# marcin-ochman/modular-slam

Hardware: AMD Instinct MI355X
Metric: ORB keypoints extracted+matched /sec, 640×480 RGB-D, 1/2/4/8 GPU; HBM GB/s vs roofline (higher is better)
Workload: dtype u8

## Files before the change

### modular-slam_amd/csrc/api.hip

```cpp
#include "context.hpp"

#include <cfloat>
#include <climits>
#include <cmath>
#include <cstdio>
#include <cstring>
#include <cstdlib>
#include <algorithm>

using namespace mslam;

static thread_local std::string g_create_error;

#define HIPCHK(c, call)                                                                                                \
    do                                                                                                                 \
    {                                                                                                                  \
        hipError_t e_ = (call);                                                                                        \
        if(e_ != hipSuccess)                                                                                           \
        {                                                                                                              \
            (c)->err = std::string(#call) + ": " + hipGetErrorString(e_);                                              \
            return MSLAM_HIP_E_RUNTIME;                                                                                \
        }                                                                                                              \
    } while(0)

// ... 290 lines not shown
void mslam_hip_default_params(mslam_hip_params* p)
{
    std::memset(p, 0, sizeof(*p));
    p->width = 640;
    p->height = 480;
    p->max_batch = 1;
    p->n_levels = 8;
    p->scale_factor = 1.2f;
    p->ini_fast_thr = 20;
    p->min_fast_thr = 7;
    p->min_node_area = 1000;
    p->max_keypoints = 8192;
    p->max_candidates = 16384;
    p->device = 0;
    p->stream = nullptr;
    p->detector = MSLAM_HIP_DETECTOR_DISTRIBUTED;
    p->n_features = 1000;
    p->edge_threshold = 31;
}

int mslam_hip_abi_version(void) { return MSLAM_HIP_ABI_VERSION; }

const char* mslam_hip_last_error(const mslam_hip_ctx* ctx) { return ctx ? ctx->err.c_str() : g_create_error.c_str(); }

void mslam_hip_destroy(mslam_hip_ctx* c)
{
    if(!c)
        return;
    if(c->stream)
        (void)hipStreamSynchronize(c->stream);
    void* bufs[] = {c->d_cells,   c->d_rs_ofs, c->d_rs_coef, c->d_rs_qt, c->d_ratio_thr, c->d_orient_w, c->d_stage,  c->d_pyr,
                    c->d_blur,    c->d_cv_ofs, c->d_cv_coef, c->d_cell_cnt, c->d_cell_kp, c->quad.cand, c->quad.cand_cnt, c->quad.sel,
                    c->quad.sel_cnt, c->quad.kp_node, c->quad.nodes_a, c->quad.nodes_b, c->quad.ncnt_a, c->quad.ncnt_b,
                    c->quad.child_cnt, c->quad.ninfo, c->quad.best, c->d_flags, c->d_hm_from, c->d_hm_out, c->d_hm_partial,
                    c->d_xyz, c->d_valid, c->d_pnp_obj, c->d_pnp_img, c->d_pnp_n, c->d_pnp_counts, c->d_pnp_hyp, c->d_pnp_out,
                    c->d_pnp_mask, c->d_blur_waves, c->d_pnp1_obj, c->d_pnp1_img, c->d_pnp1_hyp, c->d_pnp1_out,
                    c->d_pnp1_counts, c->d_pnp1_mask, c->d_mse1};
    for(void* b : bufs)
        if(b)
            (void)hipFree(b);
    if(c->h_out)
        (void)hipHostFree(c->h_out);
    if(c->h_hm)
        (void)hipHostFree(c->h_hm);
    if(c->h_stage)
        (void)hipHostFree(c->h_stage);
    if(c->match_graph)
        (void)hipGraphExecDestroy(c->match_graph);
    for(auto& e : c->detect_graph)
        if(e)
            (void)hipGraphExecDestroy(e);
    if(c->stream_m)
        (void)hipStreamSynchronize(c->stream_m);
    for(auto& o : c->out)
    {
        void* ob[] = {o.xy, o.desc, o.octave, o.angle, o.response, o.count, o.idx0, o.idx1, o.dist0, o.dist1, o.mfrom, o.mto, o.mcount};
        for(void* b : ob)
            if(b)
                (void)hipFree(b);
        if(o.ev_detect)
            (void)hipEventDestroy(o.ev_detect);
        if(o.ev_match)
            (void)hipEventDestroy(o.ev_match);
    }
    if(c->stream_m)
        (void)hipStreamDestroy(c->stream_m);
    for(auto& t : c->timers)
// ... 272 lines not shown
                              (double)B * g.slab < 4294901760.0  && (size_t)B * (p.width / 4) < (1u << 22) && p.height >= 8;
            int n_fused = fits ? 1 : 0;
            while(n_fused >= 1 && n_fused < p.n_levels && c->rs_q[n_fused] != SIZE_MAX && g.lv[n_fused].h >= 8 &&
                  (size_t)B * ((g.lv[n_fused].w + 3) / 4) < (1u << 22))
                ++n_fused;
            c->fused_levels = std::max(0, std::min(want, n_fused));
            const char* t = getenv("MSLAM_HIP_TILED_BLUR");
            c->geom.blur_tiled = c->fused_levels == p.n_levels && !(t && atoi(t) == 0) ? 1 : 0;
        }
        std::vector<BlurWave> bw;
        build_blur_waves(g, c->fused_levels, bw);
        c->blur_wpf = (int)bw.size();
        if(!bw.empty())
        {
            HIPCHK(c, dmalloc(c->d_blur_waves, bw.size()));
            HIPCHK(c, hipMemcpy(c->d_blur_waves, bw.data(), bw.size() * sizeof(BlurWave), hipMemcpyHostToDevice));
        }
    }
    HIPCHK(c, dmalloc(c->d_cell_cnt, B * g.n_cells));
    HIPCHK(c, dmalloc(c->d_cell_kp, B * g.n_cells * (size_t)kCellCap));
    QuadArgs& q = c->quad;
    HIPCHK(c, dmalloc(q.cand, B * L * cap));
    HIPCHK(c, dmalloc(q.cand_cnt, B * L));
    HIPCHK(c, dmalloc(q.sel, B * L * cap));
    HIPCHK(c, dmalloc(q.sel_cnt, B * L));
    HIPCHK(c, dmalloc(q.kp_node, B * L * cap));
    HIPCHK(c, dmalloc(q.nodes_a, B * L * cap));
    HIPCHK(c, dmalloc(q.nodes_b, B * L * cap));
    HIPCHK(c, dmalloc(q.ncnt_a, B * L * cap));
    HIPCHK(c, dmalloc(q.ncnt_b, B * L * cap));
    HIPCHK(c, dmalloc(q.child_cnt, B * L * cap * 4));
    HIPCHK(c, dmalloc(q.ninfo, B * L * cap));
    HIPCHK(c, dmalloc(q.best, B * L * cap));
    q.cell_cnt = c->d_cell_cnt;
    q.cell_kp = c->d_cell_kp;
    q.flags = c->d_flags;
    q.cand_cap = p.max_candidates;
    q.min_size = p.min_node_area;
    }

    for(auto& o : c->out)
    {
        HIPCHK(c, dmalloc(o.xy, (B + 1) * K * 2));
        HIPCHK(c, dmalloc(o.desc, (B + 1) * K * 32));
        HIPCHK(c, dmalloc(o.octave, (B + 1) * K));
        HIPCHK(c, dmalloc(o.angle, (B + 1) * K));
        HIPCHK(c, dmalloc(o.response, (B + 1) * K));
        HIPCHK(c, dmalloc(o.count, B + 1));
        HIPCHK(c, hipMemset(o.count, 0, (B + 1) * 4));
        HIPCHK(c, dmalloc(o.idx0, B * K));
        HIPCHK(c, dmalloc(o.idx1, B * K));
        HIPCHK(c, dmalloc(o.dist0, B * K));
        HIPCHK(c, dmalloc(o.dist1, B * K));
        HIPCHK(c, dmalloc(o.mfrom, B * K));
        HIPCHK(c, dmalloc(o.mto, B * K));
        HIPCHK(c, dmalloc(o.mcount, B));
        HIPCHK(c, hipMemset(o.mcount, 0, B * 4));
        HIPCHK(c, hipEventCreateWithFlags(&o.ev_detect, hipEventDisableTiming));
        HIPCHK(c, hipEventCreateWithFlags(&o.ev_match, hipEventDisableTiming));
    }
    HIPCHK(c, hipStreamCreateWithFlags(&c->stream_m, hipStreamNonBlocking));
    {
        const char* e = getenv("MSLAM_HIP_OVERLAP_MATCH");
        c->overlap_match = !(e && atoi(e) == 0);
        auto on = [](const char* name) { const char* v = getenv(name); return !v || atoi(v) != 0; };
        c->knob_mirror_results = on("MSLAM_HIP_MIRROR_RESULTS");
        c->knob_zero_copy = on("MSLAM_HIP_ZERO_COPY_FRAME");
        c->knob_match_graph = on("MSLAM_HIP_MATCH_GRAPH");
        const char* zm = getenv("MSLAM_HIP_ZERO_COPY_MAX_BYTES");
        c->zero_copy_max_bytes = zm ? (size_t)atoll(zm) : (size_t)1200000;
        const char* m = getenv("MSLAM_HIP_MATCHER");
// ... 329 lines not shown
        else if(blur_needed)
        {
            StageScope t(c, "blur", cs);
            launch_blur(c->d_pyr, c->d_blur, g, c->d_blur_waves, c->blur_wpf, f0, nf, cs);
        }
        }
        if(cv_mode && c->fused_levels < g.n_levels)
        {
            StageScope t(c, "blur", cs);
            launch_blur(c->d_pyr, c->d_blur, g, c->d_blur_waves, c->blur_wpf, f0, nf, cs);
        }
        {
            StageScope t(c, "describe", cs);
            DescArgs a{};
            a.pyr = c->d_pyr;
            a.blur = c->d_blur;
            a.sel = c->quad.sel;
            a.sel_cnt = c->quad.sel_cnt;
            a.orient_w = c->d_orient_w;
            a.cand_cap = c->p.max_candidates;
            a.max_kp = c->p.max_keypoints;
            a.xy = c->d_xy + K * 2;
            a.desc = c->d_desc + K * 32;
            a.octave = c->d_octave + K;
            a.angle = c->d_angle + K;
            a.response = c->d_response + K;
            a.count = c->d_count + 1;
            a.flags = c->d_flags;
            if(cv_mode)
            {
                a.sel_resp = reinterpret_cast<const float*>(c->quad.best);
                a.cv_mode = 1;
            }
            if(c->mirror_results && n_frames == 1)
                a.h_mirror = c->d_h_out;
            launch_describe(g, a, f0, nf, cs);
        }
        if(n_chunks > 1)
        {
            HIPCHK(c, hipEventRecord(c->ev_join[k], cs));
            HIPCHK(c, hipStreamWaitEvent(s, c->ev_join[k], 0));
        }
    }
    HIPCHK(c, hipGetLastError());
    return MSLAM_HIP_OK;
}

static int detect_prologue(mslam_hip_ctx* c)
{
    const size_t K = (size_t)c->p.max_keypoints;
    hipStream_t s = c->stream;
    if(!c->inplace_timing)
        c->timers_used = 0;
    if(c->n_last > 0)
    {
        const int prev = c->cur, nxt = prev ^ 1;
        if(c->out[nxt].match_pending)
        {
            HIPCHK(c, hipStreamWaitEvent(s, c->out[nxt].ev_match, 0));
            c->out[nxt].match_pending = false;
        }
        const size_t last = (size_t)c->n_last;
        hipLaunchKernelGGL(k_carry_prev, dim3(16), dim3(256), 0, s, reinterpret_cast<uint4*>(c->out[nxt].desc),
                           reinterpret_cast<const uint4*>(c->out[prev].desc + last * K * 32), c->out[nxt].count,
                           c->out[prev].count + last, (int)K);
        HIPCHK(c, hipGetLastError());
// ... 646 lines not shown
```

### modular-slam_amd/csrc/common.hpp

```cpp
#pragma once
#include <hip/hip_runtime.h>
#include <cstdint>
#include <cstddef>

namespace mslam
{

constexpr int kMaxLevels = 16;
constexpr int kBorder = 19;
constexpr int kCell = 64;
constexpr int kOverlap = 6;
constexpr int kCellCap = 1024;

struct LevelGeom
{
    int w, h;
    int pitch;
    int offset;
    float scale;
    int bw, bh;
    int cell_base;
    int n_cells;
    int bsx;
    int nxg, nyg;
// ... 66 lines not shown
    const uint4* qt;
    const int32_t* yofs;
    const uint32_t* ycoef;
    int frame0, n_frames;
    int quads;
    float inv_quads;
    int R;
    int need_mask;
    int exact;
};
void launch_resize_col(const ResizeColArgs& a, hipStream_t s);
void launch_fast(const uint8_t* d_pyr, const Geometry& g, const CellDesc* d_cells, uint32_t* d_cell_cnt,
                 uint32_t* d_cell_kp, int ini_thr, int min_thr, int frame0, int n_frames, hipStream_t s);
void launch_denorm_selfcheck(uint32_t* d_out, hipStream_t s);
struct QuadArgs
{
    const uint32_t* cell_cnt;
    const uint32_t* cell_kp;
    uint32_t* cand;
    uint32_t* cand_cnt;
    uint32_t* sel;
    uint32_t* sel_cnt;
    uint32_t* kp_node;
    uint2* nodes_a;
    uint2* nodes_b;
    uint32_t* ncnt_a;
    uint32_t* ncnt_b;
    uint32_t* child_cnt;
    uint32_t* ninfo;
    uint32_t* best;
    uint32_t* flags;
    int cand_cap;
    unsigned min_size;
};
void launch_quadtree(const Geometry& g, const QuadArgs& a, int frame0, int n_frames, hipStream_t s);
struct BlurK
{
    uint32_t ta[3], tb[4], tc[4];
    uint32_t t01, t23, t45, t6;
};
BlurK make_blur_k();
struct GrayBlurArgs
{
    const uint8_t* bgr;
    uint8_t* pyr;
    uint8_t* blur;
    int W, H, pitch;
    unsigned slab;
    int n_frames, frame0;
    int quads;
    float inv_quads;
    int k6;
    int waves_per_xcd;
    int blur_tiled;
    BlurK bk;
};
void launch_gray_blur(const GrayBlurArgs& a, hipStream_t s);
struct ResizeBlurArgs
{
    uint8_t* pyr;
    uint8_t* blur;
    unsigned slab;
    int src_off, sh, spitch, dst_off, dw, dh, dpitch;
    const uint4* qt;
    const int32_t* yofs;
    const uint32_t* ycoef;
// ... 17 lines not shown
    int n_lv;
    int G;
    int n_groups, groups_per_xcd;
    int frame0, n_frames;
};
bool launch_level_chain(const GrayBlurArgs& g, const ResizeBlurArgs* lv, int n_lv, int frames_per_group, int waves, int k6_max, hipStream_t s);
struct BlurWave
{
    int level;
    int item0;
    int generic;
    float inv_bsx;
};
void launch_blur(const uint8_t* d_pyr, uint8_t* d_blur, const Geometry& g, const BlurWave* d_waves, int wpf, int frame0, int n_frames,
                 hipStream_t s);
struct DescArgs
{
    const uint8_t* pyr;
    const uint8_t* blur;
    const uint32_t* sel;
    const uint32_t* sel_cnt;
    const uint32_t* orient_w;
    int cand_cap;
    int max_kp;
    float* xy;
    uint8_t* desc;
    int32_t* octave;
    float* angle;
    float* response;
    int32_t* count;
    uint32_t* flags;
    int n_frames = 0;
    const float* sel_resp = nullptr;
    uint8_t* h_mirror = nullptr;
    int cv_mode = 0;
};
void launch_describe(const Geometry& g, const DescArgs& a, int frame0, int n_frames, hipStream_t s);

struct ExactResizeArgs
{
    uint8_t* pyr;
    unsigned slab;
    int src_off, sw, sh, spitch, dst_off, dw, dh, dpitch;
    const int32_t* xofs;
    const uint32_t* xcoef;
    const int32_t* yofs;
    const uint32_t* ycoef;
    int xmin, xmax, ymin, ymax;
    int window12;
    int frame0;
};
void launch_resize_exact(const ExactResizeArgs& a, int n_frames, hipStream_t s);
struct CvSelectArgs
{
    uint32_t* cand;
    uint32_t* cand_cnt;
    uint32_t* tmp_kp;
    float* tmp_resp;
    uint32_t* sel;
    float* sel_resp;
    uint32_t* sel_cnt;
    uint32_t* flags;
    int cand_cap;
    int edge;
    int quota[kMaxLevels];
    int std_order;
// ... 46 lines not shown
```

### modular-slam_amd/csrc/k_describe.hip

```cpp
#include "common.hpp"
#include <cstdlib>
#include <type_traits>
#include "../../include/mslam_orb_pattern.h"
#include "../../include/mslam_sincos.h"

namespace mslam
{

__constant__ __attribute__((aligned(16))) float c_pattern_f[1024] = MSLAM_ORB_PATTERN_INIT;

__device__ __forceinline__ float fast_atan2_deg(float y, float x)
{
    constexpr float scale = (float)(180 / 3.1415926535897932384626433832795);
    constexpr float p1 = 0.9997878412794807f * scale, p3 = -0.3258083974640975f * scale;
    constexpr float p5 = 0.1555786518463281f * scale, p7 = -0.04432655554792128f * scale;
    const float ax = fabsf(x), ay = fabsf(y);
    const float eps = (float)2.2204460492503131e-16;
    float a, c, c2;
    if(ax >= ay)
        c = __fdiv_rn(ay, __fadd_rn(ax, eps));
    else
        c = __fdiv_rn(ax, __fadd_rn(ay, eps));
    c2 = __fmul_rn(c, c);
    a = __fadd_rn(__fmul_rn(p7, c2), p5);
    a = __fadd_rn(__fmul_rn(a, c2), p3);
    a = __fadd_rn(__fmul_rn(a, c2), p1);
    a = __fmul_rn(a, c);
    if(!(ax >= ay))
        a = __fsub_rn(90.f, a);
    if(x < 0)
        a = __fsub_rn(180.f, a);
    if(y < 0)
        a = __fsub_rn(360.f, a);
    return a;
}

__device__ __forceinline__ float poly_cos(float v)
{
    const float c1 = 0.99940307f, c2 = -0.49558072f, c3 = 0.03679168f;
    const float v2 = __fmul_rn(v, v);
    return __fadd_rn(c1, __fmul_rn(v2, __fadd_rn(c2, __fmul_rn(c3, v2))));
}
__device__ __forceinline__ float util_cos(float v)
{
    constexpr float PI = 3.14159265358979f;
    constexpr float PI_2 = PI / 2.0f, TWO_PI = 2.0f * PI, INV_TWO_PI = 1.0f / TWO_PI, THREE_PI_2 = 3.0f * PI_2;
    v = __fsub_rn(v, __fmul_rn((float)(int)floorf(__fmul_rn(v, INV_TWO_PI)), TWO_PI));
    v = (0.0f < v) ? v : -v;
    if(v < PI_2)
        return poly_cos(v);
    else if(v < PI)
        return -poly_cos(__fsub_rn(PI, v));
    else if(v < THREE_PI_2)
        return -poly_cos(__fsub_rn(v, PI));
    else
        return poly_cos(__fsub_rn(TWO_PI, v));
}
__device__ __forceinline__ float util_sin(float v)
{
    constexpr float PI_2 = 3.14159265358979f / 2.0f;
    return util_cos(__fsub_rn(PI_2, v));
}

constexpr int kPatchR = 18;
constexpr int kPatchRows = 2 * kPatchR + 1;
constexpr int kPatchRowsT = kPatchRows + 1;
constexpr int kPatchDw = 12;
#ifndef MSLAM_DISC_DW
#define MSLAM_DISC_DW 16
#endif
constexpr int kPatchDwT = 16;
constexpr int kPatchBufsT = 4;
constexpr int kPatchBufs = 5;
constexpr int kBlocksPerFrame = 32;

__device__ __forceinline__ uint32_t write_lane(uint32_t dst, uint32_t val, int sel)
{
    uint32_t keep_m0;
    asm volatile("s_mov_b32 %1, m0\n\ts_mov_b32 m0, %3\n\ts_nop 4\n\tv_writelane_b32 %0, %2, m0\n\ts_mov_b32 m0, %1"
                 : "+v"(dst), "=&s"(keep_m0)
                 : "s"(val), "s"(sel));
    return dst;
}

__device__ __forceinline__ int wave_sum_dpp(int v)
{
    v += __builtin_amdgcn_update_dpp(0, v, 0x111, 0xF, 0xF, true);
    v += __builtin_amdgcn_update_dpp(0, v, 0x112, 0xF, 0xF, true);
    v += __builtin_amdgcn_update_dpp(0, v, 0x114, 0xF, 0xE, true);
    v += __builtin_amdgcn_update_dpp(0, v, 0x118, 0xF, 0xC, true);
    v += __builtin_amdgcn_update_dpp(0, v, 0x142, 0xA, 0xF, true);
    v += __builtin_amdgcn_update_dpp(0, v, 0x143, 0xC, 0xF, true);
    return __builtin_amdgcn_readlane(v, 63);
}


__device__ __forceinline__ void wave_sum_dpp2(int a, int b, int& ra, int& rb)
{
    a += __builtin_amdgcn_update_dpp(0, a, 0x111, 0xF, 0xF, true);
    b += __builtin_amdgcn_update_dpp(0, b, 0x111, 0xF, 0xF, true);
    a += __builtin_amdgcn_update_dpp(0, a, 0x112, 0xF, 0xF, true);
    b += __builtin_amdgcn_update_dpp(0, b, 0x112, 0xF, 0xF, true);
    a += __builtin_amdgcn_update_dpp(0, a, 0x114, 0xF, 0xE, true);
    b += __builtin_amdgcn_update_dpp(0, b, 0x114, 0xF, 0xE, true);
    a += __builtin_amdgcn_update_dpp(0, a, 0x118, 0xF, 0xC, true);
    b += __builtin_amdgcn_update_dpp(0, b, 0x118, 0xF, 0xC, true);
    a += __builtin_amdgcn_update_dpp(0, a, 0x142, 0xA, 0xF, true);
    b += __builtin_amdgcn_update_dpp(0, b, 0x142, 0xA, 0xF, true);
    a += __builtin_amdgcn_update_dpp(0, a, 0x143, 0xC, 0xF, true);
    b += __builtin_amdgcn_update_dpp(0, b, 0x143, 0xC, 0xF, true);
    ra = __builtin_amdgcn_readlane(a, 63);
    rb = __builtin_amdgcn_readlane(b, 63);
}

constexpr int kBatch = 16;
typedef float f32x2 __attribute__((ext_vector_type(2)));

template <bool TILED>
__global__ __launch_bounds__(256) void k_describe(Geometry g, DescArgs a, int bpf, int kb)
{
    constexpr int kBufs = TILED ? kPatchBufsT : kPatchBufs;
    constexpr int kSlotDw = TILED ? kPatchRowsT * kPatchDwT : kPatchRows * kPatchDw;
    constexpr int kDiscDw = TILED ? MSLAM_DISC_DW : 12;
    __shared__ __attribute__((aligned(16))) uint32_t patch[4][kBufs][kSlotDw];

    const bool spread = kb < kBatch;
    const int xcd = blockIdx.x & 7, slot = spread ? (int)blockIdx.x : (int)(blockIdx.x >> 3);
    const int f_local = spread ? slot / bpf : (slot / bpf) * 8 + xcd;
    if(f_local >= a.n_frames)
        return;
    const int bx = slot % bpf;
    const size_t frame = (size_t)f_local + g.frame0;
    const int lane = threadIdx.x & 63;
    const int wave = __builtin_amdgcn_readfirstlane(threadIdx.x >> 6);

    const uint32_t* sel_cnt = a.sel_cnt + frame * g.n_levels;
    int total = 0;
    for(int l = 0; l < g.n_levels; ++l)
        total += (int)sel_cnt[l];
    if(bx == 0 && threadIdx.x == 0)
    {
        a.count[frame] = min(total, a.max_kp);
        if(total > a.max_kp)
            atomicOr(a.flags, kFlagKpOverflow);
        if(a.h_mirror)
        {
            reinterpret_cast<int32_t*>(a.h_mirror)[0] = min(total, a.max_kp);
            reinterpret_cast<uint32_t*>(a.h_mirror)[1] = __hip_atomic_load(a.flags, __ATOMIC_RELAXED, __HIP_MEMORY_SCOPE_AGENT) | (total > a.max_kp ? kFlagKpOverflow : 0u);
        }
    }
    const int n_kp = min(total, a.max_kp);

    uint32_t wu[4], wv[4];
    f32x2 patX[4], patY[4];
#pragma unroll
    for(int k = 0; k < 4; ++k)
    {
        wu[k] = a.orient_w[lane + 64 * k];
        wv[k] = a.orient_w[256 + lane + 64 * k];
        const float4 q = reinterpret_cast<const float4*>(c_pattern_f)[lane + 64 * k];
        patX[k] = f32x2{q.x, q.z};
        patY[k] = f32x2{q.y, q.w};
    }
    const uint8_t* pyr = a.pyr + frame * g.slab;
    const uint8_t* blur = a.blur + frame * g.slab;
    auto bc = [&](uint32_t v, int k) -> uint32_t { return (uint32_t)__builtin_amdgcn_readlane((int)v, k); };
    int lv_cum = 0;
    uint32_t lv_pitch = 16, lv_offset = 0, lv_scale = 0;
    {
        const int ll = min(lane, g.n_levels - 1);
        int c = lane < g.n_levels ? (int)sel_cnt[ll] : 0;
#pragma unroll
        for(int o = 1; o < kMaxLevels; o <<= 1)
        {
            const int t = __shfl_up(c, o);
            c += lane >= o ? t : 0;
        }
        lv_cum = c;
        const LevelGeom* lvp = &g.lv[0];
        lv_pitch = (uint32_t)lvp[ll].pitch;
        lv_offset = (uint32_t)lvp[ll].offset;
        lv_scale = __float_as_uint(lvp[ll].scale);
    }
    __builtin_amdgcn_s_waitcnt(0x0F70);

    constexpr int kStr = 4;
    for(int base = bx * 4 * kb + wave; base < n_kp; base += bpf * 4 * kb)
    {
        const int n_here = min(kb, (n_kp - base + kStr - 1) / kStr);

        uint32_t my_kp = 0;
        int my_level = 0;
        uint32_t my_doff = 0, my_poff = 0, my_pitch = 16, my_sh = 0, my_lut = 0;
        float my_scale = 1.f, my_resp = 0.f;
        {
            const int idx = base + lane * kStr;
            uint32_t lofs = 0;
            {
                int lvl = 0;
#pragma unroll 1
                for(int l = 0; l + 1 < g.n_levels; ++l)
                    lvl += idx >= __builtin_amdgcn_readlane(lv_cum, l) ? 1 : 0;
                my_level = lvl;
                const int prev_cum = __shfl(lv_cum, lvl > 0 ? lvl - 1 : 0);
                const int first = lvl > 0 ? prev_cum : 0;
                my_pitch = (uint32_t)__shfl((int)lv_pitch, lvl);
                lofs = (uint32_t)__shfl((int)lv_offset, lvl);
                my_scale = __uint_as_float((uint32_t)__shfl((int)lv_scale, lvl));
                my_kp = (uint32_t)(idx - first);
            }
            if(lane < n_here)
            {
                const size_t si = (frame * g.n_levels + my_level) * (size_t)a.cand_cap + my_kp;
                my_kp = a.sel[si];
                my_resp = a.sel_resp ? a.sel_resp[si] : (float)kp_score(my_kp);
                const int px = kp_x(my_kp) + kBorder, py = kp_y(my_kp) + kBorder;
                my_doff = lofs + (uint32_t)(py - 15) * my_pitch + (uint32_t)((px - 15) & ~15);
                my_sh = (uint32_t)((px - 15) & 15) | ((uint32_t)((px - kPatchR) & 15) << 4);
                if(TILED)
                {
                    const uint32_t xa = (uint32_t)((px - kPatchR) & ~15), ya = (uint32_t)(py - kPatchR);
                    my_poff = lofs + (ya & ~1u) * my_pitch + 2u * (xa & ~63u);
                    const uint32_t sum = 0x03020100u + ((xa >> 4) & 3u) * 0x01010101u;
                    my_lut = sum + (((sum + 0x7C7C7C7Cu) & 0x80808080u) >> 5);
                    my_sh |= (ya & 1u) << 8;
                }
                else
                    my_poff = lofs + (uint32_t)(py - kPatchR) * my_pitch + (uint32_t)((px - kPatchR) & ~15);
            }
        }
        __builtin_amdgcn_s_waitcnt(0x0F70);
        __builtin_amdgcn_sched_barrier(0);
        int my_m10 = 0, my_m01 = 0;
        {
            auto dma_disc = [&](int k, int buf) {
                const uint8_t* src = pyr + bc(my_doff, k);
                const uint32_t pitch = bc(my_pitch, k);
#pragma unroll
                for(int q = 0; q < 2; ++q)
                {
                    const uint32_t t = (uint32_t)lane + 64u * q;
                    if(kDiscDw == 16)
                    {
                        const uint8_t* sq = src + (size_t)(16u * q * pitch);
                        asm volatile("" : "+s"(sq));
                        if(t < 124u && (t & 3u) != 3u)
                            __builtin_amdgcn_global_load_lds(
                                (const __attribute__((address_space(1))) void*)(sq + (__umul24((uint32_t)lane >> 2, pitch) + 16u * ((uint32_t)lane & 3u))),
                                (__attribute__((address_space(3))) void*)&patch[wave][buf][q * 256], 16, 0, 0);
                    }
                    else if(t < 93u)
                    {
                        const uint32_t row = (t * 21846u) >> 16;
                        __builtin_amdgcn_global_load_lds(
                            (const __attribute__((address_space(1))) void*)(src + __umul24(row, pitch) + 16u * (t - 3u * row)),
                            (__attribute__((address_space(3))) void*)&patch[wave][buf][q * 256], 16, 0, 0);
                    }
                }
            };
            auto reduce = [&](int k, int buf) {
                const int sh = (int)(bc(my_sh, k) & 15u);
                const uint32_t* d = patch[wave][buf] + (sh >> 2);
                int m10 = 0, m01 = 0;
#pragma unroll
                for(int q = 0; q < 4; ++q)
                {
                    const int t = lane + 64 * q;
                    uint32_t x = 0x80808080u;
                    if(t < 31 * 8)
                    {
                        const uint32_t* e = d + (t >> 3) * kDiscDw + (t & 7);
                        x = __builtin_amdgcn_alignbyte(e[1], e[0], sh & 3);
                    }
                    x ^= 0x80808080u;
                    m10 = __builtin_amdgcn_sdot4((int)x, (int)wu[q], m10, false);
                    m01 = __builtin_amdgcn_sdot4((int)x, (int)wv[q], m01, false);
                }
                int t10, t01;
                wave_sum_dpp2(m10, m01, t10, t01);
                my_m10 = (int)write_lane((uint32_t)my_m10, (uint32_t)t10, k);
                my_m01 = (int)write_lane((uint32_t)my_m01, (uint32_t)t01, k);
            };
            constexpr int kDepthA = kBufs - 1;
#pragma unroll
            for(int i = 0; i < kDepthA; ++i)
                if(i < n_here)
                    dma_disc(i, i);
            for(int k = 0; k < n_here; ++k)
            {
                const int younger = min(kDepthA, n_here - 1 - k);
                if(k + kDepthA < n_here)
                    dma_disc(k + kDepthA, (k + kDepthA) % kBufs);
                if(younger >= 4)
                    __builtin_amdgcn_s_waitcnt(0x0F70 | 8);
                else if(younger == 3)
                    __builtin_amdgcn_s_waitcnt(0x0F70 | 6);
                else if(younger == 2)
                    __builtin_amdgcn_s_waitcnt(0x0F70 | 4);
                else if(younger == 1)
                    __builtin_amdgcn_s_waitcnt(0x0F70 | 2);
                else
                    __builtin_amdgcn_s_waitcnt(0x0F70 | 0);
                __builtin_amdgcn_wave_barrier();
                reduce(k, k % kBufs);
                __builtin_amdgcn_wave_barrier();
            }
        }

        auto dma_patch = [&](int k, int buf) {
// ... 21 lines not shown
                {
                    const uint32_t r3 = ((uint32_t)lane * 21846u) >> 16, c3 = (uint32_t)lane - 3u * r3;
                    const uint32_t lo = (__builtin_amdgcn_ubfe(lut, 8u * c3, 8u) << 4) + (__umul24(r3 & ~1u, pitch) + ((r3 & 1u) << 6));
#pragma unroll
                    for(int q = 0; q < 2; ++q)
                    {
                        const uint8_t* bq = bsrc + (size_t)(20u * q * pitch);
                        asm volatile("" : "+s"(bq));
                        if((uint32_t)lane < (q == 0 ? 60u : (uint32_t)(kPatchRowsT * 3 - 60)))
                            __builtin_amdgcn_global_load_lds((const __attribute__((address_space(1))) void*)(bq + lo),
                                                             (__attribute__((address_space(3))) void*)&patch[wave][buf][q * 240], 16, 0, 0);
                    }
                }
                return;
            }
            bsrc += shp > 11u ? 12 : 0;
#pragma unroll
            for(int q = 0; q < 2; ++q)
            {
                const uint32_t t = (uint32_t)lane + 64u * q;
                const uint32_t row = (t * 21846u) >> 16;
                if(t < (uint32_t)(kPatchRows * 3))
                    __builtin_amdgcn_global_load_lds(
                        (const __attribute__((address_space(1))) void*)(bsrc + __umul24(row, pitch) + 16u * (t - 3u * row)),
                        (__attribute__((address_space(3))) void*)&patch[wave][buf][q * 256], 16, 0, 0);
            }
        };
        constexpr int kDepth = kBufs - 1;
#pragma unroll
        for(int i = 0; i < kDepth; ++i)
            if(i < n_here)
                dma_patch(i, i);

        float my_ca = 0.f, my_sa = 0.f, my_angle = 0.f, my_ox = 0.f, my_oy = 0.f;
        if(lane < n_here)
        {
            my_angle = fast_atan2_deg((float)my_m01, (float)my_m10);
            if(a.cv_mode)
            {
                const float rad = __fmul_rn(my_angle, (float)(3.1415926535897932384626433832795 / 180.f));
                mslam_sincos_f32(rad, &my_sa, &my_ca);
            }
            else
            {
                const float rad = (float)((double)my_angle * 3.14159265358979323846 / 180.0);
                my_ca = util_cos(rad);
                my_sa = util_sin(rad);
            }
            const float fx = (float)(kp_x(my_kp) + kBorder), fy = (float)(kp_y(my_kp) + kBorder);
            my_ox = my_level == 0 ? fx : __fmul_rn(fx, my_scale);
            my_oy = my_level == 0 ? fy : __fmul_rn(fy, my_scale);
        }

        uint32_t desc_lo = 0, desc_hi = 0;
        {
            auto describe = [&](int k, int buf) {
                const float ca = __builtin_bit_cast(float, __builtin_amdgcn_readlane(__builtin_bit_cast(int, my_ca), k));
                const float sa = __builtin_bit_cast(float, __builtin_amdgcn_readlane(__builtin_bit_cast(int, my_sa), k));
                f32x2 ca2 = f32x2{ca, ca}, sa2 = f32x2{sa, sa};
                asm volatile("" : "+v"(ca2), "+v"(sa2));
                const f32x2 magic = f32x2{12582912.f, 12582912.f};
                const uint32_t lp_lds = (uint32_t)(size_t)(__attribute__((address_space(3))) void*)patch[wave][buf];
                const uint32_t shk = bc(my_sh, k);
                const uint32_t shp = (shk >> 4) & 15u, odd_row = (shk >> 8) & 1u;
                unsigned long long bits[4];
                auto sample = [&](auto wide) {
                    constexpr bool WIDE = decltype(wide)::value;
                    constexpr uint32_t P = WIDE ? 64u : 48u;
                    const uint32_t ctr = lp_lds + (uint32_t)(kPatchR * P + kPatchR) + (TILED ? shp + odd_row * P : shp <= 11u ? shp : shp - 12u) -
                                         (WIDE ? P * 0x4B400000u : P * 0x00400000u) - 0x4B400000u;
// ... 61 lines not shown
            a.angle[o] = my_angle;
            a.response[o] = my_resp;
        }
        if(a.h_mirror)
        {
            const size_t K = (size_t)a.max_kp;
            uint8_t* h = a.h_mirror + 16;
            if(lane < 4 * n_here)
                reinterpret_cast<uint2*>(h + K * 8 + (size_t)(base + (lane >> 2) * kStr) * 32)[lane & 3] = make_uint2(desc_lo, desc_hi);
            if(lane < n_here)
            {
                const size_t o = (size_t)(base + lane * kStr);
                reinterpret_cast<float2*>(h)[o] = make_float2(my_ox, my_oy);
                reinterpret_cast<int32_t*>(h + K * 40)[o] = my_level;
                reinterpret_cast<float*>(h + K * 44)[o] = my_angle;
                reinterpret_cast<float*>(h + K * 48)[o] = my_resp;
            }
        }
    }
}

void launch_describe(const Geometry& g, const DescArgs& a, int frame0, int n_frames, hipStream_t s)
{
    Geometry gg = g;
    gg.frame0 = frame0;
    DescArgs aa = a;
    aa.n_frames = n_frames;
    static const int bpf_env = [] { const char* e = getenv("MSLAM_DESC_BPF"); return e ? atoi(e) : 0; }();
    static const int kb_env = [] { const char* e = getenv("MSLAM_DESC_KB_SMALL"); return e ? atoi(e) : 0; }();
    const bool small = n_frames < 8;
    const int kb = small ? (kb_env >= 1 && kb_env <= kBatch ? kb_env : 4) : kBatch;
    const int bpf = bpf_env ? bpf_env : small ? 4 * kBlocksPerFrame : kBlocksPerFrame;
    const unsigned grid = kb < kBatch ? (unsigned)n_frames * (unsigned)bpf : (unsigned)((n_frames + 7) / 8) * 8u * (unsigned)bpf;
    if(g.blur_tiled)
        hipLaunchKernelGGL(k_describe<true>, dim3(grid), dim3(256), 0, s, gg, aa, bpf, kb);
    else
        hipLaunchKernelGGL(k_describe<false>, dim3(grid), dim3(256), 0, s, gg, aa, bpf, kb);
}

}
```

### modular-slam_amd/csrc/k_quadtree.hip

```cpp
#include "common.hpp"
#include <cstdlib>

namespace mslam
{

constexpr int QT = 512;
constexpr int kSmallKp = 512, kSmallQT = 256;
constexpr int kMidKp = 1024, kMidQT = 512;
constexpr int kLdsKp = 2048;
constexpr int kMaxCellsPerLevel = 2048;
constexpr int kBigNodes = 4096;
constexpr int kBigKp = 12288;
constexpr int kBigMinPixels = 400000;
constexpr int kMaxInitNodes = 64;
constexpr int kMaxPasses = 40;

struct Scan
{
    uint32_t wsum[QT / 64];
};

__device__ __forceinline__ uint32_t wave_incl_scan(uint32_t v)
{
    int x = (int)v;
    x += __builtin_amdgcn_update_dpp(0, x, 0x111, 0xF, 0xF, true);
    x += __builtin_amdgcn_update_dpp(0, x, 0x112, 0xF, 0xF, true);
    x += __builtin_amdgcn_update_dpp(0, x, 0x114, 0xF, 0xE, true);
    x += __builtin_amdgcn_update_dpp(0, x, 0x118, 0xF, 0xC, true);
    x += __builtin_amdgcn_update_dpp(0, x, 0x142, 0xA, 0xF, true);
    x += __builtin_amdgcn_update_dpp(0, x, 0x143, 0xC, 0xF, true);
    return (uint32_t)x;
}

// ... 63 lines not shown
__device__ __forceinline__ uint2 pack_node(int bx, int by, int ex, int ey)
{
    return make_uint2((uint32_t)bx | ((uint32_t)by << 16), (uint32_t)ex | ((uint32_t)ey << 16));
}

struct LdsStore
{
    using idx_t = uint16_t;
    using info_t = uint8_t;
    static constexpr bool kLds = true;
    static constexpr bool kCandCopy = true;
    static constexpr uint32_t kNodeCap = 0;
    static __device__ __forceinline__ void cc_zero(uint32_t* cc, uint32_t pos) { cc[2 * pos] = 0, cc[2 * pos + 1] = 0; }
    static __device__ __forceinline__ void cc_add(uint32_t* cc, uint32_t pos, int c) { atomicAdd(&cc[2 * pos + (c >> 1)], 1u << (16 * (c & 1))); }
    static __device__ __forceinline__ uint32_t cc_get(const uint32_t* cc, uint32_t pos, int c) { return (cc[2 * pos + (c >> 1)] >> (16 * (c & 1))) & 0xFFFFu; }
};
struct BigStore : LdsStore
{
    static constexpr bool kCandCopy = false;
    static constexpr uint32_t kNodeCap = kBigNodes;
};
struct GlobalStore
{
    using idx_t = uint32_t;
    using info_t = uint32_t;
    static constexpr bool kLds = false;
    static constexpr bool kCandCopy = false;
    static constexpr uint32_t kNodeCap = 0;
    static __device__ __forceinline__ void cc_zero(uint32_t* cc, uint32_t pos) { cc[4 * pos] = 0, cc[4 * pos + 1] = 0, cc[4 * pos + 2] = 0, cc[4 * pos + 3] = 0; }
    static __device__ __forceinline__ void cc_add(uint32_t* cc, uint32_t pos, int c) { atomicAdd(&cc[4 * pos + c], 1u); }
    static __device__ __forceinline__ uint32_t cc_get(const uint32_t* cc, uint32_t pos, int c) { return ld_atomic(&cc[4 * pos + c]); }
};

template <class S, int NT>
__device__ __forceinline__ bool quad_run(const Geometry& g, const QuadArgs& a, const LevelGeom& lv, size_t frame,
                                         size_t slot, int tid, uint32_t N, int n_cells, const uint32_t* cell_off,
                                         uint32_t* cand, uint32_t* g_cand, typename S::idx_t* kp_node, uint2* nodes,
                                         uint2* nodes2, typename S::idx_t* ncnt, typename S::idx_t* ncnt2,
                                         typename S::info_t* ninfo, typename S::idx_t* nbase, uint32_t* cc,
                                         uint32_t* best, uint32_t* sel, Scan& scan, Scan& scan2, uint32_t* init_cnt,
                                         uint32_t* init_pos, uint32_t& sh_n)
{
    using idx_t = typename S::idx_t;
    constexpr uint32_t kNoNode = (uint32_t)(idx_t)~(idx_t)0;

    const uint32_t* ckp = a.cell_kp + (frame * g.n_cells + lv.cell_base) * (size_t)kCellCap;
    for(uint32_t j = tid; j < N; j += NT)
    {
        int lo = 0, hi = n_cells - 1;
        while(lo < hi)
        {
            const int mid = (lo + hi + 1) >> 1;
            if(cell_off[mid] <= j)
                lo = mid;
            else
                hi = mid - 1;
        }
        const uint32_t v = ckp[(size_t)lo * kCellCap + (j - cell_off[lo])];
        cand[j] = v;
        if(S::kCandCopy)
            g_cand[j] = v;
    }
    __syncthreads();

    const int n_init = lv.nxg * lv.nyg;
    if(tid < kMaxInitNodes)
// ... 141 lines not shown
            }
            else
                np = T + (uint32_t)nbase[pos];
            kp_node[k] = (idx_t)np;
        }
        __syncthreads();
        {
            uint2* t = nodes; nodes = nodes2; nodes2 = t;
            idx_t* u = ncnt; ncnt = ncnt2; ncnt2 = u;
        }
        const uint32_t n2 = T + U;
        const bool same = n2 == n;
        n = n2;
        if(same)
        {
            converged = true;
            break;
        }
    }
    if(!converged && n > 0 && tid == 0)
        atomicOr(a.flags, kFlagQuadNoConverge);

    for(uint32_t pos = tid; pos < n; pos += NT)
        best[pos] = 0;
    __syncthreads();
    for(uint32_t k = tid; k < N; k += NT)
    {
        const uint32_t pos = kp_node[k];
        if(pos == kNoNode)
            continue;
        atomicMax(&best[pos], ((uint32_t)kp_score(cand[k]) << 24) | (0xFFFFFFu - k));
    }
    __syncthreads();
    for(uint32_t pos = tid; pos < n; pos += NT)
    {
        const uint32_t k = 0xFFFFFFu - ((S::kLds ? best[pos] : ld_atomic(&best[pos])) & 0xFFFFFFu);
        sel[pos] = cand[k];
    }
    if(tid == 0)
        a.sel_cnt[slot] = n;
    return true;
}

template <int NT>
__device__ __forceinline__ uint32_t quad_cell_offsets(const uint32_t* ccnt, int n_cells, uint32_t* cell_off, Scan& scan)
{
    const int tid = threadIdx.x;
    uint32_t running = 0;
    for(int base = 0; base < n_cells; base += NT)
    {
        const int i = base + tid;
        const uint32_t v = i < n_cells ? ccnt[i] : 0u;
        uint32_t tot;
        const uint32_t ex = block_excl_scan<NT>(v, scan, tot);
        if(i < n_cells)
            cell_off[i] = running + ex;
        running += tot;
    }
    if(tid == 0)
        cell_off[n_cells] = running;
    __syncthreads();
    return running;
}

__device__ __forceinline__ int quad_class(uint32_t N, int n_cells, unsigned classes)
{
    if((classes & 1u) && N <= (uint32_t)kSmallKp && n_cells <= 2 * kSmallKp - 1)
        return 0;
    if((classes & 2u) && N <= (uint32_t)kMidKp && n_cells <= 2 * kMidKp - 1)
        return 1;
    return 2;
}
template <int KP, int NT, int CLS>
// ... 148 lines not shown
```

Baseline: 626.1 million.

## Compute keypoint orientation in quadtree emit stage instead of describe kernel

Moves the intensity-centroid orientation computation out of the describe kernel and into the quadtree selection's final emit step. Each lane reads its selected keypoint's 31x31 disc straight from the pyramid with vector loads and writes the angle to a new sel_angle buffer. The describe kernel gains an ORIENT template flag and, in non-cv mode, skips its disc DMA and moment reduction and just loads the precomputed angle. This removes a cooperative LDS staging pass from describe, but the quadtree kernel now does per-lane, uncoalesced global loads and has to be recompiled with more code.

Result: slower. 395.4 million (median of 2 runs) (-36.8%).

```diff
diff --git a/modular-slam_amd/csrc/api.hip b/modular-slam_amd/csrc/api.hip
--- a/modular-slam_amd/csrc/api.hip
+++ b/modular-slam_amd/csrc/api.hip
@@ -346,7 +346,7 @@
     void* bufs[] = {c->d_cells,   c->d_rs_ofs, c->d_rs_coef, c->d_rs_qt, c->d_ratio_thr, c->d_orient_w, c->d_stage,  c->d_pyr,
                     c->d_blur,    c->d_cv_ofs, c->d_cv_coef, c->d_cell_cnt, c->d_cell_kp, c->quad.cand, c->quad.cand_cnt, c->quad.sel,
                     c->quad.sel_cnt, c->quad.kp_node, c->quad.nodes_a, c->quad.nodes_b, c->quad.ncnt_a, c->quad.ncnt_b,
-                    c->quad.child_cnt, c->quad.ninfo, c->quad.best, c->d_flags, c->d_hm_from, c->d_hm_out, c->d_hm_partial,
+                    c->quad.child_cnt, c->quad.ninfo, c->quad.best, c->quad.sel_angle, c->d_flags, c->d_hm_from, c->d_hm_out, c->d_hm_partial,
                     c->d_xyz, c->d_valid, c->d_pnp_obj, c->d_pnp_img, c->d_pnp_n, c->d_pnp_counts, c->d_pnp_hyp, c->d_pnp_out,
                     c->d_pnp_mask, c->d_blur_waves, c->d_pnp1_obj, c->d_pnp1_img, c->d_pnp1_hyp, c->d_pnp1_out,
                     c->d_pnp1_counts, c->d_pnp1_mask, c->d_mse1};
@@ -685,11 +685,14 @@
     HIPCHK(c, dmalloc(q.child_cnt, B * L * cap * 4));
     HIPCHK(c, dmalloc(q.ninfo, B * L * cap));
     HIPCHK(c, dmalloc(q.best, B * L * cap));
+    HIPCHK(c, dmalloc(q.sel_angle, B * L * cap));
     q.cell_cnt = c->d_cell_cnt;
     q.cell_kp = c->d_cell_kp;
     q.flags = c->d_flags;
     q.cand_cap = p.max_candidates;
     q.min_size = p.min_node_area;
+    q.pyr = c->d_pyr;
+    q.orient_w = c->d_orient_w;
     }
 
     for(auto& o : c->out)
@@ -1085,6 +1088,8 @@
                 a.sel_resp = reinterpret_cast<const float*>(c->quad.best);
                 a.cv_mode = 1;
             }
+            else
+                a.sel_angle = c->quad.sel_angle;
             if(c->mirror_results && n_frames == 1)
                 a.h_mirror = c->d_h_out;
             launch_describe(g, a, f0, nf, cs);
diff --git a/modular-slam_amd/csrc/common.hpp b/modular-slam_amd/csrc/common.hpp
--- a/modular-slam_amd/csrc/common.hpp
+++ b/modular-slam_amd/csrc/common.hpp
@@ -122,6 +122,9 @@
     uint32_t* flags;
     int cand_cap;
     unsigned min_size;
+    const uint8_t* pyr;
+    const uint32_t* orient_w;
+    float* sel_angle;
 };
 void launch_quadtree(const Geometry& g, const QuadArgs& a, int frame0, int n_frames, hipStream_t s);
 struct BlurK
@@ -205,6 +208,7 @@
     uint32_t* flags;
     int n_frames = 0;
     const float* sel_resp = nullptr;
+    const float* sel_angle = nullptr;
     uint8_t* h_mirror = nullptr;
     int cv_mode = 0;
 };
diff --git a/modular-slam_amd/csrc/k_describe.hip b/modular-slam_amd/csrc/k_describe.hip
--- a/modular-slam_amd/csrc/k_describe.hip
+++ b/modular-slam_amd/csrc/k_describe.hip
@@ -1,4 +1,5 @@
 #include "common.hpp"
+#include "orient.hpp"
 #include <cstdlib>
 #include <type_traits>
 #include "../../include/mslam_orb_pattern.h"
@@ -8,32 +9,6 @@
 {
 
 __constant__ __attribute__((aligned(16))) float c_pattern_f[1024] = MSLAM_ORB_PATTERN_INIT;
-
-__device__ __forceinline__ float fast_atan2_deg(float y, float x)
-{
-    constexpr float scale = (float)(180 / 3.1415926535897932384626433832795);
-    constexpr float p1 = 0.9997878412794807f * scale, p3 = -0.3258083974640975f * scale;
-    constexpr float p5 = 0.1555786518463281f * scale, p7 = -0.04432655554792128f * scale;
-    const float ax = fabsf(x), ay = fabsf(y);
-    const float eps = (float)2.2204460492503131e-16;
-    float a, c, c2;
-    if(ax >= ay)
-        c = __fdiv_rn(ay, __fadd_rn(ax, eps));
-    else
-        c = __fdiv_rn(ax, __fadd_rn(ay, eps));
-    c2 = __fmul_rn(c, c);
-    a = __fadd_rn(__fmul_rn(p7, c2), p5);
-    a = __fadd_rn(__fmul_rn(a, c2), p3);
-    a = __fadd_rn(__fmul_rn(a, c2), p1);
-    a = __fmul_rn(a, c);
-    if(!(ax >= ay))
-        a = __fsub_rn(90.f, a);
-    if(x < 0)
-        a = __fsub_rn(180.f, a);
-    if(y < 0)
-        a = __fsub_rn(360.f, a);
-    return a;
-}
 
 __device__ __forceinline__ float poly_cos(float v)
 {
@@ -74,15 +49,6 @@
 constexpr int kPatchBufs = 5;
 constexpr int kBlocksPerFrame = 32;
 
-__device__ __forceinline__ uint32_t write_lane(uint32_t dst, uint32_t val, int sel)
-{
-    uint32_t keep_m0;
-    asm volatile("s_mov_b32 %1, m0\n\ts_mov_b32 m0, %3\n\ts_nop 4\n\tv_writelane_b32 %0, %2, m0\n\ts_mov_b32 m0, %1"
-                 : "+v"(dst), "=&s"(keep_m0)
-                 : "s"(val), "s"(sel));
-    return dst;
-}
-
 __device__ __forceinline__ int wave_sum_dpp(int v)
 {
     v += __builtin_amdgcn_update_dpp(0, v, 0x111, 0xF, 0xF, true);
@@ -95,28 +61,10 @@
 }
 
 
-__device__ __forceinline__ void wave_sum_dpp2(int a, int b, int& ra, int& rb)
-{
-    a += __builtin_amdgcn_update_dpp(0, a, 0x111, 0xF, 0xF, true);
-    b += __builtin_amdgcn_update_dpp(0, b, 0x111, 0xF, 0xF, true);
-    a += __builtin_amdgcn_update_dpp(0, a, 0x112, 0xF, 0xF, true);
-    b += __builtin_amdgcn_update_dpp(0, b, 0x112, 0xF, 0xF, true);
-    a += __builtin_amdgcn_update_dpp(0, a, 0x114, 0xF, 0xE, true);
-    b += __builtin_amdgcn_update_dpp(0, b, 0x114, 0xF, 0xE, true);
-    a += __builtin_amdgcn_update_dpp(0, a, 0x118, 0xF, 0xC, true);
-    b += __builtin_amdgcn_update_dpp(0, b, 0x118, 0xF, 0xC, true);
-    a += __builtin_amdgcn_update_dpp(0, a, 0x142, 0xA, 0xF, true);
-    b += __builtin_amdgcn_update_dpp(0, b, 0x142, 0xA, 0xF, true);
-    a += __builtin_amdgcn_update_dpp(0, a, 0x143, 0xC, 0xF, true);
-    b += __builtin_amdgcn_update_dpp(0, b, 0x143, 0xC, 0xF, true);
-    ra = __builtin_amdgcn_readlane(a, 63);
-    rb = __builtin_amdgcn_readlane(b, 63);
-}
-
 constexpr int kBatch = 16;
 typedef float f32x2 __attribute__((ext_vector_type(2)));
 
-template <bool TILED>
+template <bool TILED, bool ORIENT>
 __global__ __launch_bounds__(256) void k_describe(Geometry g, DescArgs a, int bpf, int kb)
 {
     constexpr int kBufs = TILED ? kPatchBufsT : kPatchBufs;
@@ -151,13 +99,16 @@
     }
     const int n_kp = min(total, a.max_kp);
 
-    uint32_t wu[4], wv[4];
+    uint32_t wu[4] = {0, 0, 0, 0}, wv[4] = {0, 0, 0, 0};
     f32x2 patX[4], patY[4];
 #pragma unroll
     for(int k = 0; k < 4; ++k)
     {
-        wu[k] = a.orient_w[lane + 64 * k];
-        wv[k] = a.orient_w[256 + lane + 64 * k];
+        if(ORIENT)
+        {
+            wu[k] = a.orient_w[lane + 64 * k];
+            wv[k] = a.orient_w[256 + lane + 64 * k];
+        }
         const float4 q = reinterpret_cast<const float4*>(c_pattern_f)[lane + 64 * k];
         patX[k] = f32x2{q.x, q.z};
         patY[k] = f32x2{q.y, q.w};
@@ -192,7 +143,7 @@
         uint32_t my_kp = 0;
         int my_level = 0;
         uint32_t my_doff = 0, my_poff = 0, my_pitch = 16, my_sh = 0, my_lut = 0;
-        float my_scale = 1.f, my_resp = 0.f;
+        float my_scale = 1.f, my_resp = 0.f, my_angle = 0.f;
         {
             const int idx = base + lane * kStr;
             uint32_t lofs = 0;
@@ -214,6 +165,8 @@
                 const size_t si = (frame * g.n_levels + my_level) * (size_t)a.cand_cap + my_kp;
                 my_kp = a.sel[si];
                 my_resp = a.sel_resp ? a.sel_resp[si] : (float)kp_score(my_kp);
+                if(!ORIENT)
+                    my_angle = a.sel_angle[si];
                 const int px = kp_x(my_kp) + kBorder, py = kp_y(my_kp) + kBorder;
                 my_doff = lofs + (uint32_t)(py - 15) * my_pitch + (uint32_t)((px - 15) & ~15);
                 my_sh = (uint32_t)((px - 15) & 15) | ((uint32_t)((px - kPatchR) & 15) << 4);
@@ -232,6 +185,7 @@
         __builtin_amdgcn_s_waitcnt(0x0F70);
         __builtin_amdgcn_sched_barrier(0);
         int my_m10 = 0, my_m01 = 0;
+        if constexpr(ORIENT)
         {
             auto dma_disc = [&](int k, int buf) {
                 const uint8_t* src = pyr + bc(my_doff, k);
@@ -272,9 +226,7 @@
                         const uint32_t* e = d + (t >> 3) * kDiscDw + (t & 7);
                         x = __builtin_amdgcn_alignbyte(e[1], e[0], sh & 3);
                     }
-                    x ^= 0x80808080u;
-                    m10 = __builtin_amdgcn_sdot4((int)x, (int)wu[q], m10, false);
-                    m01 = __builtin_amdgcn_sdot4((int)x, (int)wv[q], m01, false);
+                    disc_dot4(x, wu[q], wv[q], m10, m01);
                 }
                 int t10, t01;
                 wave_sum_dpp2(m10, m01, t10, t01);
@@ -362,10 +314,11 @@
             if(i < n_here)
                 dma_patch(i, i);
 
-        float my_ca = 0.f, my_sa = 0.f, my_angle = 0.f, my_ox = 0.f, my_oy = 0.f;
+        float my_ca = 0.f, my_sa = 0.f, my_ox = 0.f, my_oy = 0.f;
         if(lane < n_here)
         {
-            my_angle = fast_atan2_deg((float)my_m01, (float)my_m10);
+            if(ORIENT)
+                my_angle = ic_angle_deg(my_m01, my_m10);
             if(a.cv_mode)
             {
                 const float rad = __fmul_rn(my_angle, (float)(3.1415926535897932384626433832795 / 180.f));
@@ -493,10 +446,15 @@
     const int kb = small ? (kb_env >= 1 && kb_env <= kBatch ? kb_env : 4) : kBatch;
     const int bpf = bpf_env ? bpf_env : small ? 4 * kBlocksPerFrame : kBlocksPerFrame;
     const unsigned grid = kb < kBatch ? (unsigned)n_frames * (unsigned)bpf : (unsigned)((n_frames + 7) / 8) * 8u * (unsigned)bpf;
-    if(g.blur_tiled)
-        hipLaunchKernelGGL(k_describe<true>, dim3(grid), dim3(256), 0, s, gg, aa, bpf, kb);
+    const bool orient = a.sel_angle == nullptr;
+    if(g.blur_tiled && orient)
+        hipLaunchKernelGGL((k_describe<true, true>), dim3(grid), dim3(256), 0, s, gg, aa, bpf, kb);
+    else if(g.blur_tiled)
+        hipLaunchKernelGGL((k_describe<true, false>), dim3(grid), dim3(256), 0, s, gg, aa, bpf, kb);
+    else if(orient)
+        hipLaunchKernelGGL((k_describe<false, true>), dim3(grid), dim3(256), 0, s, gg, aa, bpf, kb);
     else
-        hipLaunchKernelGGL(k_describe<false>, dim3(grid), dim3(256), 0, s, gg, aa, bpf, kb);
-}
-
-}
+        hipLaunchKernelGGL((k_describe<false, false>), dim3(grid), dim3(256), 0, s, gg, aa, bpf, kb);
+}
+
+}
diff --git a/modular-slam_amd/csrc/k_quadtree.hip b/modular-slam_amd/csrc/k_quadtree.hip
--- a/modular-slam_amd/csrc/k_quadtree.hip
+++ b/modular-slam_amd/csrc/k_quadtree.hip
@@ -1,4 +1,5 @@
 #include "common.hpp"
+#include "orient.hpp"
 #include <cstdlib>
 
 namespace mslam
@@ -128,6 +129,67 @@
     static __device__ __forceinline__ uint32_t cc_get(const uint32_t* cc, uint32_t pos, int c) { return ld_atomic(&cc[4 * pos + c]); }
 };
 
+template <class S, int NT>
+__device__ __forceinline__ void quad_emit(const Geometry& g, const QuadArgs& a, const LevelGeom& lv, size_t frame, size_t slot,
+                                          int tid, uint32_t n, const uint32_t* cand, const uint32_t* best, uint32_t* sel)
+{
+    typedef uint32_t u32x4 __attribute__((ext_vector_type(4)));
+    const int lane = tid & 63;
+    const uint8_t* plane = a.pyr + frame * g.slab + (size_t)lv.offset;
+    const uint32_t pitch = (uint32_t)lv.pitch;
+    float* sel_angle = a.sel_angle + slot * (size_t)a.cand_cap;
+    n = (uint32_t)__builtin_amdgcn_readfirstlane((int)n);
+
+    for(uint32_t base = (uint32_t)__builtin_amdgcn_readfirstlane(tid & ~63); base < n; base += NT)
+    {
+        const uint32_t pos = base + (uint32_t)lane;
+        uint32_t my_kp = 0;
+        if(pos < n)
+        {
+            const uint32_t k = 0xFFFFFFu - ((S::kLds ? best[pos] : ld_atomic(&best[pos])) & 0xFFFFFFu);
+            my_kp = cand[k];
+            sel[pos] = my_kp;
+        }
+        my_kp = pos < n ? my_kp : (uint32_t)__builtin_amdgcn_readfirstlane((int)my_kp);
+        const uint32_t x0 = (uint32_t)(kp_x(my_kp) + kBorder - 15), y0 = (uint32_t)(kp_y(my_kp) + kBorder - 15);
+        const uint8_t* src = plane + (size_t)(y0 * pitch + (x0 & ~15u));
+        const bool s2 = (x0 & 8u) != 0u, s1 = (x0 & 4u) != 0u;
+        const uint32_t b = x0 & 3u;
+        auto load = [&](int r, u32x4* d) {
+            const u32x4* p = reinterpret_cast<const u32x4*>(src + (size_t)r * pitch);
+            d[0] = p[0];
+            d[1] = p[1];
+            d[2] = p[2];
+        };
+        int m10 = 0, m01 = 0;
+        auto reduce = [&](int r, const u32x4* d) {
+            const uint32_t D[12] = {d[0].x, d[0].y, d[0].z, d[0].w, d[1].x, d[1].y, d[1].z, d[1].w, d[2].x, d[2].y, d[2].z, d[2].w};
+            uint32_t E[10], F[9];
+#pragma unroll
+            for(int j = 0; j < 10; ++j)
+                E[j] = s2 ? D[j + 2] : D[j];
+#pragma unroll
+            for(int j = 0; j < 9; ++j)
+                F[j] = s1 ? E[j + 1] : E[j];
+#pragma unroll
+            for(int i = 0; i < 8; ++i)
+                disc_dot4(__builtin_amdgcn_alignbyte(F[i + 1], F[i], b), a.orient_w[8 * r + i], a.orient_w[256 + 8 * r + i], m10, m01);
+        };
+        u32x4 d0[3], d1[3];
+        load(0, d0);
+#pragma unroll 1
+        for(int r = 0; r < 30; r += 2)
+        {
+            load(r + 1, d1);
+            reduce(r, d0);
+            load(r + 2, d0);
+            reduce(r + 1, d1);
+        }
+        reduce(30, d0);
+        if(pos < n)
+            sel_angle[pos] = ic_angle_deg(m01, m10);
+    }
+}
 template <class S, int NT>
 __device__ __forceinline__ bool quad_run(const Geometry& g, const QuadArgs& a, const LevelGeom& lv, size_t frame,
                                          size_t slot, int tid, uint32_t N, int n_cells, const uint32_t* cell_off,
@@ -335,13 +397,9 @@
         atomicMax(&best[pos], ((uint32_t)kp_score(cand[k]) << 24) | (0xFFFFFFu - k));
     }
     __syncthreads();
-    for(uint32_t pos = tid; pos < n; pos += NT)
-    {
-        const uint32_t k = 0xFFFFFFu - ((S::kLds ? best[pos] : ld_atomic(&best[pos])) & 0xFFFFFFu);
-        sel[pos] = cand[k];
-    }
     if(tid == 0)
         a.sel_cnt[slot] = n;
+    quad_emit<S, NT>(g, a, lv, frame, slot, tid, n, cand, best, sel);
     return true;
 }
 
diff --git a/modular-slam_amd/csrc/orient.hpp b/modular-slam_amd/csrc/orient.hpp
--- /dev/null
+++ b/modular-slam_amd/csrc/orient.hpp
@@ -0,0 +1,69 @@
+#pragma once
+#include "common.hpp"
+
+namespace mslam
+{
+
+__device__ __forceinline__ float fast_atan2_deg(float y, float x)
+{
+    constexpr float scale = (float)(180 / 3.1415926535897932384626433832795);
+    constexpr float p1 = 0.9997878412794807f * scale, p3 = -0.3258083974640975f * scale;
+    constexpr float p5 = 0.1555786518463281f * scale, p7 = -0.04432655554792128f * scale;
+    const float ax = fabsf(x), ay = fabsf(y);
+    const float eps = (float)2.2204460492503131e-16;
+    float a, c, c2;
+    if(ax >= ay)
+        c = __fdiv_rn(ay, __fadd_rn(ax, eps));
+    else
+        c = __fdiv_rn(ax, __fadd_rn(ay, eps));
+    c2 = __fmul_rn(c, c);
+    a = __fadd_rn(__fmul_rn(p7, c2), p5);
+    a = __fadd_rn(__fmul_rn(a, c2), p3);
+    a = __fadd_rn(__fmul_rn(a, c2), p1);
+    a = __fmul_rn(a, c);
+    if(!(ax >= ay))
+        a = __fsub_rn(90.f, a);
+    if(x < 0)
+        a = __fsub_rn(180.f, a);
+    if(y < 0)
+        a = __fsub_rn(360.f, a);
+    return a;
+}
+
+__device__ __forceinline__ float ic_angle_deg(int m01, int m10) { return fast_atan2_deg((float)m01, (float)m10); }
+
+__device__ __forceinline__ void disc_dot4(uint32_t x, uint32_t wu, uint32_t wv, int& m10, int& m01)
+{
+    x ^= 0x80808080u;
+    m10 = __builtin_amdgcn_sdot4((int)x, (int)wu, m10, false);
+    m01 = __builtin_amdgcn_sdot4((int)x, (int)wv, m01, false);
+}
+
+__device__ __forceinline__ uint32_t write_lane(uint32_t dst, uint32_t val, int sel)
+{
+    uint32_t keep_m0;
+    asm volatile("s_mov_b32 %1, m0\n\ts_mov_b32 m0, %3\n\ts_nop 4\n\tv_writelane_b32 %0, %2, m0\n\ts_mov_b32 m0, %1"
+                 : "+v"(dst), "=&s"(keep_m0)
+                 : "s"(val), "s"(sel));
+    return dst;
+}
+
+__device__ __forceinline__ void wave_sum_dpp2(int a, int b, int& ra, int& rb)
+{
+    a += __builtin_amdgcn_update_dpp(0, a, 0x111, 0xF, 0xF, true);
+    b += __builtin_amdgcn_update_dpp(0, b, 0x111, 0xF, 0xF, true);
+    a += __builtin_amdgcn_update_dpp(0, a, 0x112, 0xF, 0xF, true);
+    b += __builtin_amdgcn_update_dpp(0, b, 0x112, 0xF, 0xF, true);
+    a += __builtin_amdgcn_update_dpp(0, a, 0x114, 0xF, 0xE, true);
+    b += __builtin_amdgcn_update_dpp(0, b, 0x114, 0xF, 0xE, true);
+    a += __builtin_amdgcn_update_dpp(0, a, 0x118, 0xF, 0xC, true);
+    b += __builtin_amdgcn_update_dpp(0, b, 0x118, 0xF, 0xC, true);
+    a += __builtin_amdgcn_update_dpp(0, a, 0x142, 0xA, 0xF, true);
+    b += __builtin_amdgcn_update_dpp(0, b, 0x142, 0xA, 0xF, true);
+    a += __builtin_amdgcn_update_dpp(0, a, 0x143, 0xC, 0xF, true);
+    b += __builtin_amdgcn_update_dpp(0, b, 0x143, 0xC, 0xF, true);
+    ra = __builtin_amdgcn_readlane(a, 63);
+    rb = __builtin_amdgcn_readlane(b, 63);
+}
+
+}
```
